# itxtx/normalizing-flows-study

Hardware: AMD Instinct MI355X
Metric: log_prob samples/sec/GPU + test-NLL match; RealNVP d=2 and MAF d=63 (higher is better)
Workload: dtype fp32

## Files before the change

normalizing-flows-study_amd/csrc/nfx_affine_kernel.h:

```cpp
#pragma once
#include <type_traits>
#include <utility>

#include "nfx_common.h"

namespace nfx {

__host__ __device__ constexpr int up4(int v) { return (v + 3) & ~3; }

struct AffineLayout {
    int d, HT, KS1;
    int w1, b1, w2, b2, w3, b3, net, mask, total;
    int s;
};

constexpr uint32_t kAffineLiveElide = 0x100u;
struct AffineSplit {
    int w1, b1, b2, w3, b3, w2s, net, mask, ok, total;
};

__host__ __device__ constexpr AffineSplit affine_split(int d, int HT) {
    AffineSplit S{};
    int o = 0;
    S.w1 = o; o += HT * ((d + 1) / 2) * 64;
    S.b1 = o; o += HT * 32;
    S.b2 = o; o += HT * 32;
    S.w3 = o; o += d * HT * 32;
// ... 101 lines not shown
                const f32x4 w = wg[a_quad(a_tile(hto, kt, HT), rq) * 64];
#pragma unroll
                for (int rr = 0; rr < 4; ++rr) {
                    a0 = mfma32(w[rr], h1[kt][0][4 * rq + rr], a0);
                    if constexpr (TILES == 2) a1 = mfma32(w[rr], h1[kt][1][4 * rq + rr], a1);
                }
            }
        }
#pragma unroll
        for (int j = 0; j < D; ++j) {
            const f32x16 w3 = load_bias16(P + L.w3 + (j * HT + hto) * 32, h);
#pragma unroll
            for (int r = 0; r < 16; ++r) {
                part[j][0] = fmaf(w3[r], trelu(a0[r]), part[j][0]);
                if constexpr (TILES == 2) part[j][1] = fmaf(w3[r], trelu(a1[r]), part[j][1]);
            }
        }
    }
#pragma unroll
    for (int j = 0; j < D; ++j)
        res[j] = tclamp(halves_sum(part[j][0], part[j][1]) + P[L.b3 + j], -10.f, 10.f);
}

#ifndef NFX_SPLIT_TERMS
#define NFX_SPLIT_TERMS 6
#endif
typedef __bf16 bf16x8 __attribute__((ext_vector_type(8)));
typedef uint32_t u32x4 __attribute__((ext_vector_type(4)));

__device__ __forceinline__ f32x16 mfma_bf16(u32x4 a, u32x4 b, f32x16 c) {
    return __builtin_amdgcn_mfma_f32_32x32x16_bf16(__builtin_bit_cast(bf16x8, a), __builtin_bit_cast(bf16x8, b), c,
                                                    0, 0, 0);
}

__device__ __forceinline__ void split3(float x, uint32_t& u0, uint32_t& u1, uint32_t& u2) {
    u0 = __float_as_uint(x) & 0xffff0000u;
    const float r1 = x - __uint_as_float(u0);
    u1 = __float_as_uint(r1) & 0xffff0000u;
    u2 = __float_as_uint(r1 - __uint_as_float(u1));
}

__device__ __forceinline__ uint32_t pack_bf16(uint32_t lo, uint32_t hi) {
    return __builtin_amdgcn_perm(hi, lo, 0x07060302u);
}

__device__ __forceinline__ void split_block(const f32x16& a, int half, u32x4 (&xp)[3]) {
#pragma unroll
    for (int q = 0; q < 4; ++q) {
        uint32_t l0, l1, l2, h0, h1, h2;
        split3(a[8 * half + 2 * q], l0, l1, l2);
        split3(a[8 * half + 2 * q + 1], h0, h1, h2);
        xp[0][q] = pack_bf16(l0, h0);
        xp[1][q] = pack_bf16(l1, h1);
        xp[2][q] = pack_bf16(l2, h2);
    }
}

template <class F, int... I>
__device__ __forceinline__ void static_for_seq(F&& f, std::integer_sequence<int, I...>) {
    (f(std::integral_constant<int, I>{}), ...);
}
template <int N, class F>
__device__ __forceinline__ void static_for(F&& f) {
    static_for_seq(f, std::make_integer_sequence<int, N>{});
}

#if NFX_SPLIT_TERMS == 8
constexpr int kSplitTermW[8] = {2, 1, 2, 1, 0, 1, 0, 0}, kSplitTermX[8] = {1, 2, 0, 1, 2, 0, 1, 0};
#else
constexpr int kSplitTermW[6] = {2, 1, 0, 1, 0, 0}, kSplitTermX[6] = {0, 1, 2, 0, 1, 0};
#endif

template <int HT, int D, int TILES, bool LIVE>
__device__ __forceinline__ void affine_nets_split_pipe(const float* __restrict__ S, const AffineSplit& SL,
                                                       const float (&xb)[2][(D + 1) / 2], float (&sv)[D],
                                                       float (&bv)[D], uint32_t live_idx) {
    constexpr int KS1 = (D + 1) / 2;
    constexpr int NJ = LIVE ? (D + 1) / 2 : D;
    constexpr int NS = 2 * TILES;
    constexpr int KB = 2 * HT;
    constexpr int NT = NFX_SPLIT_TERMS;
    constexpr int NM = NT * HT;
    constexpr int NG = KB * NM;
    constexpr int NFI = 16 * HT;
    constexpr int NQ = 3 * HT;
    constexpr int WG0 = (NM - NQ) / 2;
    constexpr int L1G = (KB - 2) * NM;
    constexpr int L1P = L1G >= 2 ? L1G - 2 : 0;
    constexpr int HB0 = NM / 2;
    const int lane = lane_id(), h = lane >> 5;

    const float* Sn[NS];
    const u32x4* w2n[NS];
    f32x16 h1[NS][HT];
// ... 565 lines not shown
```

normalizing-flows-study_amd/csrc/nfx_made.hip:

```cpp
#include "nfx_made_kernel.h"
#include "nfx_made_wide_kernel.h"
#include <atomic>
#include <cstdlib>

#include "nfx_made_seqs_kernel.h"
#include "nfx_pack.h"

namespace nfx {

__global__ void made_pack_kernel(NfxMlpRaw net, int d, int H, float* packed) {
    const int HT = (H + 31) / 32;
    const MadeLayout L = made_layout(d, HT);
    const int Hp = L.Hp, G1 = 4 * L.NKC;
    for (int i = blockIdx.x * blockDim.x + threadIdx.x; i < L.total; i += gridDim.x * blockDim.x) {
        if (i >= L.s_deg) continue;
        float v = 0.f;
        if (i < L.b1) {
            int t = i - L.w1, rr = t & 3, lane = (t >> 2) & 63, g = (t >> 8) % G1, ht = (t >> 8) / G1;
            int row = 32 * ht + (lane & 31), col = 2 * (4 * g + rr) + (lane >> 5);
            v = (row < H && col < d) ? mlp_weight(net, 0, d, row, col) : 0.f;
        } else if (i < L.w2) {
            int row = acc_vec_row(i - L.b1);
            v = row < H ? mlp_bias(net, 0, row) : 0.f;
        } else if (i < L.b2 || (i >= L.w3 && i < L.b3)) {
            const int layer = i < L.b2 ? 1 : 2;
            const ATileElem e = a_tile_elem(i - (layer == 1 ? L.w2 : L.w3));
            int row = 32 * (e.tile / HT) + e.row, col = 32 * (e.tile % HT) + e.k;
            v = (row < H && col < H) ? mlp_weight(net, layer, H, row, col) : 0.f;
// ... 85 lines not shown
        int off, word, ext;
        if (gi < n1) {
            const int ht = gi / (4 * L.NKC), g = gi % (4 * L.NKC);
            off = L.w1 + gi * 256;
            word = L.nk1 + ht;
            ext = g / 4 + 1;
        } else if (gi < n1 + 2 * n23) {
            const int t = (gi - n1) % n23, layer = (gi - n1) / n23;
            off = (layer == 0 ? L.w2 : L.w3) + t * 256;
            word = (layer == 0 ? L.nk2 : L.nk3) + t / (HT * 4);
            ext = (t % (HT * 4)) / 4 + 1;
        } else {
            const int t = gi - n1 - 2 * n23;
            off = L.w4 + t * 256;
            word = L.nk4 + t / (2 * HT * 4);
            ext = (t % (HT * 4)) / 4 + 1;
        }
        const f32x4 v = *reinterpret_cast<const f32x4*>(packed + off + 4 * lane);
        const bool nzl = v[0] != 0.f || v[1] != 0.f || v[2] != 0.f || v[3] != 0.f;
        if (__ballot(nzl) != 0 && lane == 0) atomicMax(&nk[word], ext);
    }
}

template <int HT>
made_seqs_kernel_t made_seqs_pick_ht(int variant, bool logp) {
    if (variant == NFX_MAF_FORWARD) return made_seqs_kernel<HT, NFX_MAF_FORWARD, false>;
    return logp ? made_seqs_kernel<HT, NFX_IAF_INVERSE, true> : made_seqs_kernel<HT, NFX_IAF_INVERSE, false>;
}
template made_seqs_kernel_t made_seqs_pick_ht<1>(int, bool);
template made_seqs_kernel_t made_seqs_pick_ht<2>(int, bool);

template <int HT, int VAR>
static made_seq_kernel_t seq_var() {
    return made_seq_kernel<HT, VAR>;
}

template <int HT>
made_seq_kernel_t made_seq_pick_ht(int variant) {
    return variant == NFX_MAF_FORWARD ? seq_var<HT, NFX_MAF_FORWARD>() : seq_var<HT, NFX_IAF_INVERSE>();
}
template made_seq_kernel_t made_seq_pick_ht<1>(int);
template made_seq_kernel_t made_seq_pick_ht<2>(int);
template made_seq_kernel_t made_seq_pick_ht<3>(int);
template made_seq_kernel_t made_seq_pick_ht<4>(int);

static made_par_kernel_t pick_par(int HT, bool wlds, int variant) {
    return pick_range<1, 4>(HT, [=](auto HT_) { return made_pick_ht<HT_()>(wlds, variant); });
}

static made_par_kernel_t pick_tile(int HT, bool wlds, int variant, bool logp) {
    return pick_range<1, 4>(HT, [=](auto HT_) { return made_tile_pick_ht<HT_()>(wlds, variant, logp); });
}

static made_seq_kernel_t pick_seq(int HT, int variant) {
    return pick_range<1, 4>(HT, [=](auto HT_) { return made_seq_pick_ht<HT_()>(variant); });
}

int made_big_launch(const float* packed, const float* in, float* out, float* log_det, int64_t B, int d, int H,
                    int variant, int accumulate, hipStream_t s);

constexpr size_t kLdsBytes = 160 * 1024;
constexpr int kTileMaxD = 64;

}

using namespace nfx;

extern "C" size_t nfx_made_packed_floats(int d, int H) {
    if (d <= 0 || H <= 0) return 0;
    return (size_t)made_layout(d, (H + 31) / 32).total;
}

namespace nfx {
int made_pack_seqp(int d, int H, float* packed, hipStream_t s);
static int made_pack_seq(int d, int H, float* packed, hipStream_t s) {
    const int HT = (H + 31) / 32;
    if (HT > 2) return NFX_OK;
    if (HT == 1) made_seqs_image_kernel<1><<<64, 256, 0, s>>>(packed, d, H);
    else made_seqs_image_kernel<2><<<64, 256, 0, s>>>(packed, d, H);
    int rc = check_launch("made_seqs_image_kernel");
    if (rc) return rc;
    if (HT == 1) made_seqs_chunk_kernel<1><<<1, 64, 0, s>>>(packed, d, H);
    else made_seqs_chunk_kernel<2><<<1, 64, 0, s>>>(packed, d, H);
    rc = check_launch("made_seqs_chunk_kernel");
    if (rc) return rc;
    return made_pack_seqp(d, H, packed, s);
}
}

extern "C" int nfx_made_pack_parallel(const NfxMlpRaw* net, int d, int H, float* packed, void* stream) {
    if (!net || !packed) return set_error(NFX_EINVAL, "made_pack: null pointer");
    if (d <= 0 || d > 4096 || H <= 0 || H > 256)
        return set_error(NFX_EUNSUPPORTED, "made_pack: d=%d H=%d outside d<=4096, H<=256", d, H);
    if (net->n_layers != 4) return set_error(NFX_EINVAL, "made_pack: MADE has 4 masked layers (got %d)", net->n_layers);
    for (int l = 0; l < 4; ++l)
        if (!net->w[l]) return set_error(NFX_EINVAL, "made_pack: layer %d weight is null", l);
    const int total = (int)nfx_made_packed_floats(d, H);
    int blocks = (total + 255) / 256;
    if (blocks > 2048) blocks = 2048;
    made_pack_kernel<<<blocks, 256, 0, (hipStream_t)stream>>>(*net, d, H, packed);
    int rc = check_launch("made_pack_kernel");
    if (rc) return rc;
    made_live_kernel<<<1, kLiveThreads, 0, (hipStream_t)stream>>>(*net, d, H, packed);
    rc = check_launch("made_live_kernel");
    if (rc) return rc;
    {
        const int HT = (H + 31) / 32;
        const MadeLayout L = made_layout(d, HT);
        const int groups = HT * 4 * L.NKC + 2 * HT * HT * 4 + L.NJ * 2 * HT * 4;
        made_extent_kernel<<<(groups + 3) / 4, 256, 0, (hipStream_t)stream>>>(d, H, packed);
    }
    return check_launch("made_extent_kernel");
}

extern "C" int nfx_made_pack_sequential(int d, int H, float* packed, void* stream) {
    if (!packed) return set_error(NFX_EINVAL, "made_pack_sequential: null pointer");
    if (d <= 0 || d > 4096 || H <= 0 || H > 256)
        return set_error(NFX_EUNSUPPORTED, "made_pack_sequential: d=%d H=%d outside d<=4096, H<=256", d, H);
    return made_pack_seq(d, H, packed, (hipStream_t)stream);
}

extern "C" int nfx_made_pack(const NfxMlpRaw* net, int d, int H, float* packed, void* stream) {
    const int rc = nfx_made_pack_parallel(net, d, H, packed, stream);
    if (rc) return rc;
    return made_pack_seq(d, H, packed, (hipStream_t)stream);
}

namespace nfx {
int made_seqw_launch(const float* packed, const float* in, float* out, float* log_det, int64_t B, int d, int H,
                     int variant, int accumulate, float* logp, double* partials, double* sums, bool fused,
                     int* grid_out, hipStream_t s);
int made_seqp_launch(const float* packed, const float* in, float* out, float* log_det, int64_t B, int d, int H,
                     int variant, int accumulate, float* logp, double* partials, double* sums, bool fused,
                     hipStream_t s);
}

static std::atomic<int>& made_seq_policy() {
    static std::atomic<int> v{[] {
        const char* e = getenv("NFX_MADE_SEQ_POLICY");
        return e ? atoi(e) : NFX_MADE_SEQ_AUTO;
    }()};
    return v;
}

namespace nfx {
int made_seq_policy_get() { return made_seq_policy().load(std::memory_order_relaxed); }
}

static bool tile_path(int d, int HT, int variant) {
    return (variant == NFX_MAF_INVERSE || variant == NFX_IAF_FORWARD) && d > 0 && d <= kTileMaxD && HT >= 1 && HT <= 4;
}

struct TileConfig {
    int nw;
    bool wlds;
    size_t lds;
};
static TileConfig tile_config(const MadeLayout& L, int64_t ntiles, bool fused) {
    int nw = 8;
    if (!fused && ntiles < 4 * (int64_t)num_cus()) nw = (int)((ntiles + num_cus() - 1) / num_cus());
    const size_t wbytes = (size_t)L.par_total * sizeof(float);
    const size_t tiles = nw * 32 * (size_t)kTileStride * sizeof(float);
    const bool wlds = nw == 8 && wbytes + tiles <= kLdsBytes;
    return {nw, wlds, (wlds ? wbytes : 0) + tiles};
}

static int made_launch(const float* packed, const float* in, float* out, float* log_det, int64_t B,
                       int d, int H, int variant, int accumulate, float* logp, double* sums,
                       void* workspace, hipStream_t s) {
    const bool fused = sums != nullptr;
    if (B < 0 || d <= 0 || H <= 0) return set_error(NFX_EINVAL, "made_affine: bad shape");
    if (d > 4096 || H > 256) return set_error(NFX_EUNSUPPORTED, "made_affine: d=%d H=%d outside d<=4096, H<=256", d, H);
    if (variant < NFX_MAF_INVERSE || variant > NFX_IAF_INVERSE)
        return set_error(NFX_EINVAL, "made_affine: unknown variant %d", variant);
    const int HT = (H + 31) / 32;
    if (HT > 4) {
        if (fused) return set_error(NFX_EUNSUPPORTED, "made_affine_logprob: no fused log_prob for H=%d > 128", H);
        if (B == 0) return NFX_OK;
        if (!packed || !in || !out || !log_det) return set_error(NFX_EINVAL, "made_affine: null pointer");
        if (in == out) return set_error(NFX_EINVAL, "made_affine: in and out must not alias");
        return made_big_launch(packed, in, out, log_det, B, d, H, variant, accumulate, s);
    }
    const MadeLayout L = made_layout(d, HT);
// ... 5 lines not shown
        return set_error(NFX_EUNSUPPORTED,
                         "made_affine_logprob: fused log_prob needs MAF inverse with d <= %d or H <= 64, "
                         "or IAF inverse with H <= 64", kTileMaxD);
    if (fused && B > 0 && (!logp || !workspace)) return set_error(NFX_EINVAL, "made_affine_logprob: null logp/workspace");
    if (B == 0) return fused ? gauss_finish(reinterpret_cast<double*>(workspace), 0, sums, 0, s) : NFX_OK;
    if (!packed || !in || !out || !log_det) return set_error(NFX_EINVAL, "made_affine: null pointer");
    if (in == out) return set_error(NFX_EINVAL, "made_affine: in and out must not alias");
    double* partials = reinterpret_cast<double*>(workspace);
    if (wide) {
        const int64_t nchunks = (B + 63) / 64;
        const int nw = nchunks < (int64_t)kWideWaves * num_cus() ? 4 : kWideWaves;
        const size_t lds_nw = (size_t)wide_lds(L, HT, nw).total * sizeof(float);
        made_par_kernel_t k = HT == 1 ? made_wide_pick_ht<1>(variant, fused, nw) : made_wide_pick_ht<2>(variant, fused, nw);
        int rc = prepare_lds((const void*)k, lds_nw);
        if (rc) return rc;
        int grid = resident_grid((const void*)k, 64 * nw, lds_nw, (nchunks + nw - 1) / nw);
        if (grid > kMaxPartials) grid = kMaxPartials;
        k<<<grid, 64 * nw, lds_nw, s>>>(packed, in, out, log_det, B, d, accumulate, nchunks, logp, partials,
                                        sums, gauss_const(d));
        return check_launch("made_wide_kernel");
    }
    if (tile_path(d, HT, variant)) {
        const int64_t ntiles = (B + 31) / 32;
        const TileConfig c = tile_config(L, ntiles, fused);
        made_par_kernel_t k = pick_tile(HT, c.wlds, variant, fused);
        if (!k) return set_error(NFX_EUNSUPPORTED, "made_affine: no kernel for H=%d", H);
        int rc = prepare_lds((const void*)k, c.lds);
        if (rc) return rc;
        int grid = resident_grid((const void*)k, 64 * c.nw, c.lds, (ntiles + c.nw - 1) / c.nw);
        if (grid > kMaxPartials) grid = kMaxPartials;
        k<<<grid, 64 * c.nw, c.lds, s>>>(packed, in, out, log_det, B, d, accumulate, ntiles, logp, partials, sums,
                                         gauss_const(d));
        return check_launch("made_tile_kernel");
    }
    if (variant == NFX_MAF_INVERSE || variant == NFX_IAF_FORWARD) {
        const size_t wbytes = (size_t)L.par_total * sizeof(float);
        const size_t stage8 = 8 * (size_t)kStageFloats * sizeof(float);
        const bool wlds = wbytes + stage8 <= kLdsBytes;
        made_par_kernel_t k = pick_par(HT, wlds, variant);
        if (!k) return set_error(NFX_EUNSUPPORTED, "made_affine: no kernel for H=%d", H);
        const int threads = wlds ? 512 : 256;
        const size_t lds = wlds ? wbytes + stage8 : 4 * (size_t)kStageFloats * sizeof(float);
        int rc = prepare_lds((const void*)k, lds);
        if (rc) return rc;
        const int64_t nchunks = (B + 63) / 64;
        const int nw = threads / 64;
        const int grid = resident_grid((const void*)k, threads, lds, (nchunks + nw - 1) / nw);
        k<<<grid, threads, lds, s>>>(packed, in, out, log_det, B, d, accumulate, nchunks, nullptr, nullptr, nullptr,
// ... 47 lines not shown
                                       float* logp, double* sums, void* workspace, int64_t B, int d,
                                       int H, int variant, int accumulate, void* stream) {
    if (!sums) return set_error(NFX_EINVAL, "made_affine_logprob: null sums");
    return made_launch(packed, in, out, log_det, B, d, H, variant, accumulate, logp, sums, workspace,
                       (hipStream_t)stream);
}

extern "C" int nfx_made_sample_supported(int d, int H, int variant) {
    return (H > 0 && tile_path(d, (H + 31) / 32, variant) && variant == NFX_IAF_FORWARD) ? 1 : 0;
}

extern "C" int nfx_made_affine_sample(const float* packed, uint64_t seed, uint64_t* rng_state, float* z, float* x,
                                      float* log_det, int64_t B, int d, int H, void* stream) {
    if (B < 0 || d <= 0 || H <= 0) return set_error(NFX_EINVAL, "made_affine_sample: bad shape");
    if (!nfx_made_sample_supported(d, H, NFX_IAF_FORWARD))
        return set_error(NFX_EUNSUPPORTED, "made_affine_sample: d=%d H=%d outside the tile kernel (d <= %d, H <= 128)",
                         d, H, kTileMaxD);
    if (B == 0) return NFX_OK;
    if (!packed || !rng_state || !z || !x || !log_det) return set_error(NFX_EINVAL, "made_affine_sample: null pointer");
    if (z == x) return set_error(NFX_EINVAL, "made_affine_sample: z and x must not alias");
    const int HT = (H + 31) / 32;
    const MadeLayout L = made_layout(d, HT);
    const int64_t ntiles = (B + 31) / 32;
    const TileConfig c = tile_config(L, ntiles, false);
    made_sample_kernel_t k =
        pick_range<1, 4>(HT, [=](auto HT_) { return made_tile_sample_pick_ht<HT_()>(c.wlds); });
    int rc = prepare_lds((const void*)k, c.lds);
    if (rc) return rc;
    int grid = resident_grid((const void*)k, 64 * c.nw, c.lds, (ntiles + c.nw - 1) / c.nw);
    if (grid > kMaxPartials) grid = kMaxPartials;
    k<<<grid, 64 * c.nw, c.lds, (hipStream_t)stream>>>(packed, nullptr, x, log_det, B, d, 0, ntiles, nullptr, nullptr,
                                                       nullptr, 0.f, MadeDraw{seed, rng_state, z});
    return check_launch("made_tile_kernel");
}
```

normalizing-flows-study_amd/csrc/nfx_made_kernel.h:

```cpp
#pragma once
#include "nfx_common.h"
#include "nfx_rng.h"

namespace nfx {

struct MadeLayout {
    int d, HT, Hp, NKC, NJ;
    int w1, b1, w2, b2, w3, b3, w4, b4;
    int par_total;
    int s_w1t, s_b1, s_w2, s_b2, s_w3, s_b3, s_w4, s_b4, s_deg;
    int nk1, nk2, nk3, nk4, tsafe;
    int t4, t3, t2, t1;
    int rimg;
    int sw1, sw4, sb4;
    int ctab;
    int ps, pw4, pw1, pb4, pw23, ptb, ptab;
    int total;
};

__host__ __device__ constexpr int made_up4(int v) { return (v + 3) & ~3; }

__host__ __device__ constexpr int seqs_w4_stride(int Hp) { return 2 * Hp + 4; }
constexpr int kSeqsPadRows = 64;
__host__ __device__ constexpr int seqs_max_chunks(int d, int Hp) { return d / 8 + 2 * Hp + 8; }
constexpr int kSeqpMaxS = 16;
__host__ __device__ constexpr int seqp_slots(int d, int HT) {
    return (HT <= 2 && d <= 64 * kSeqpMaxS) ? (d + 63) / 64 : 0;
}
__host__ __device__ constexpr int seqp_max_chunks(int d, int Hp) { return (d + 63) / 64 + 3 * Hp + 4; }

__host__ __device__ constexpr MadeLayout made_layout(int d, int HT) {
    MadeLayout L{};
    L.d = d;
    L.HT = HT;
    L.Hp = 32 * HT;
    L.NKC = (d + 31) / 32;
    L.NJ = (d + 31) / 32;
    int o = 0;
    L.w1 = o; o += HT * 4 * L.NKC * 256;
    L.b1 = o; o += HT * 32;
    L.w2 = o; o += HT * HT * 1024;
    L.b2 = o; o += HT * 32;
    L.w3 = o; o += HT * HT * 1024;
    L.b3 = o; o += HT * 32;
    L.w4 = o; o += L.NJ * 2 * HT * 1024;
    L.b4 = o; o += L.NJ * 2 * 32;
    L.par_total = o;
    L.s_w1t = o; o += made_up4(d * L.Hp);
    L.s_b1 = o; o += L.Hp;
    L.s_w2 = o; o += L.Hp * L.Hp;
    L.s_b2 = o; o += L.Hp;
    L.s_w3 = o; o += L.Hp * L.Hp;
// ... 10 lines not shown
    L.t4 = o; o += HT * 2 * L.NJ * 1024;
    L.t3 = o; o += HT * HT * 1024;
    L.t2 = o; o += HT * HT * 1024;
    L.t1 = o; o += L.NKC * HT * 1024;
    L.rimg = o; o += HT <= 2 ? 2 * L.Hp * L.Hp + 5 * L.Hp : 0;
    o = made_up4(o);
    const int rows = HT <= 2 ? d + kSeqsPadRows : 0;
    L.sw1 = o; o += made_up4(rows * L.Hp);
    L.sw4 = o; o += made_up4(rows * seqs_w4_stride(L.Hp));
    L.sb4 = o; o += made_up4(2 * rows);
    L.ctab = o; o += HT <= 2 ? 8 * seqs_max_chunks(d, L.Hp) : 0;
    const int PS = seqp_slots(d, HT);
    L.ps = PS;
    L.pw4 = o; o += L.Hp * ((PS + 1) / 2) * 256;
    L.pw1 = o; o += L.Hp * ((PS + 3) / 4) * 256;
    L.pb4 = o; o += PS * 128;
    L.pw23 = o; o += PS ? 2 * L.Hp * L.Hp : 0;
    L.ptb = o; o += PS ? 4 * L.Hp : 0;
    L.ptab = o; o += PS ? 16 * seqp_max_chunks(d, L.Hp) : 0;
    L.total = o;
    return L;
}

constexpr int kStageStride = 33;
constexpr int kTileStride = 65;
constexpr int kStageFloats = 64 * kStageStride;

template <int VAR>
__device__ __forceinline__ float made_affine(float xv, float mu, float al, float& acc) {
#pragma clang fp contract(off)
    if constexpr (VAR == NFX_MAF_INVERSE) {
        const float a = tclamp(al, -3.f, 3.f);
        acc = acc + a;
        const float z = (xv - mu) * exp_fast(-a);
        return nonfinite(z) ? 0.f : z;
    } else {
        const float a = tclamp(al, -2.f, 2.f);
        const float m = tclamp(mu, -10.f, 10.f);
        acc = acc + a;
        const float y = xv * exp_fast(a) + m;
        return nonfinite(y) ? xv : y;
    }
}

__device__ __forceinline__ void stage_in(const float* __restrict__ in, int64_t base, int d, int64_t B,
                                         int dim0, float* st) {
// ... 604 lines not shown
```

normalizing-flows-study_amd/csrc/nfx_tile.h:

```cpp
#pragma once

#include <hip/hip_runtime.h>

namespace nfx {

__host__ __device__ constexpr int crow(int r, int h) { return (r & 3) + 8 * (r >> 2) + 4 * h; }
__host__ __device__ constexpr int creg(int row) { return (row & 3) + 4 * (row >> 3); }
__host__ __device__ constexpr int chalf(int row) { return (row >> 2) & 1; }

struct RowCol {
    int row, col;
};

struct ATileElem {
    int tile, row, k;
};
__host__ __device__ constexpr ATileElem a_tile_elem(int t) {
    const int rr = t & 3, lane = (t >> 2) & 63, rq = (t >> 8) & 3;
    return {t >> 10, lane & 31, crow(4 * rq + rr, lane >> 5)};
}
__host__ __device__ constexpr int a_tile(int ot, int kt, int NK) { return ot * NK + kt; }
__host__ __device__ constexpr int a_quad(int tile, int rq) { return tile * 4 + rq; }

__host__ __device__ constexpr RowCol a1_elem(int t, int KS1) {
    const int lane = t & 63, ks = (t >> 6) % KS1, ht = (t >> 6) / KS1;
    return {32 * ht + (lane & 31), 2 * ks + (lane >> 5)};
}

__host__ __device__ constexpr int acc_vec_row(int t) { return 32 * (t >> 5) + crow(t & 15, (t >> 4) & 1); }

__host__ __device__ constexpr RowCol acc_dump_elem(int t) { return {crow(t >> 6, (t >> 5) & 1), t & 31}; }
__host__ __device__ constexpr int acc_dump_index(int row, int col) {
    return creg(row) * 64 + chalf(row) * 32 + col;
}
__host__ __device__ constexpr RowCol lane_dump_elem(int t) { return {crow(t & 15, (t >> 9) & 1), (t >> 4) & 31}; }

namespace tile_check {
constexpr bool crow_round_trips() {
    for (int row = 0; row < 32; ++row)
        if (crow(creg(row), chalf(row)) != row) return false;
    for (int r = 0; r < 16; ++r)
        for (int h = 0; h < 2; ++h)
            if (creg(crow(r, h)) != r || chalf(crow(r, h)) != h) return false;
    return true;
}
constexpr bool a_tile_visits_all() {
    bool seen[32 * 32] = {};
    for (int t = 0; t < 1024; ++t) {
        const ATileElem e = a_tile_elem(t);
        if (e.tile != 0 || e.row < 0 || e.row > 31 || e.k < 0 || e.k > 31 || seen[e.row * 32 + e.k]) return false;
        seen[e.row * 32 + e.k] = true;
    }
    return true;
}
constexpr bool a_tile_encode_inverts() {
    for (int t = 0; t < 3 * 1024; ++t) {
        const ATileElem e = a_tile_elem(t);
        const int r = creg(e.k), lane = e.row + 32 * chalf(e.k);
        if ((a_quad(e.tile, r >> 2) * 64 + lane) * 4 + (r & 3) != t) return false;
    }
// ... 21 lines not shown
```

Before: 1.649 billion.

## Add bf16x3 split-MFMA tile kernel for MADE with pre-split weight image

```diff
diff --git a/normalizing-flows-study_amd/csrc/nfx_affine_kernel.h b/normalizing-flows-study_amd/csrc/nfx_affine_kernel.h
--- a/normalizing-flows-study_amd/csrc/nfx_affine_kernel.h
+++ b/normalizing-flows-study_amd/csrc/nfx_affine_kernel.h
@@ -3,6 +3,7 @@
 #include <utility>
 
 #include "nfx_common.h"
+#include "nfx_split.h"
 
 namespace nfx {
 
@@ -150,39 +151,6 @@
         res[j] = tclamp(halves_sum(part[j][0], part[j][1]) + P[L.b3 + j], -10.f, 10.f);
 }
 
-#ifndef NFX_SPLIT_TERMS
-#define NFX_SPLIT_TERMS 6
-#endif
-typedef __bf16 bf16x8 __attribute__((ext_vector_type(8)));
-typedef uint32_t u32x4 __attribute__((ext_vector_type(4)));
-
-__device__ __forceinline__ f32x16 mfma_bf16(u32x4 a, u32x4 b, f32x16 c) {
-    return __builtin_amdgcn_mfma_f32_32x32x16_bf16(__builtin_bit_cast(bf16x8, a), __builtin_bit_cast(bf16x8, b), c,
-                                                    0, 0, 0);
-}
-
-__device__ __forceinline__ void split3(float x, uint32_t& u0, uint32_t& u1, uint32_t& u2) {
-    u0 = __float_as_uint(x) & 0xffff0000u;
-    const float r1 = x - __uint_as_float(u0);
-    u1 = __float_as_uint(r1) & 0xffff0000u;
-    u2 = __float_as_uint(r1 - __uint_as_float(u1));
-}
-
-__device__ __forceinline__ uint32_t pack_bf16(uint32_t lo, uint32_t hi) {
-    return __builtin_amdgcn_perm(hi, lo, 0x07060302u);
-}
-
-__device__ __forceinline__ void split_block(const f32x16& a, int half, u32x4 (&xp)[3]) {
-#pragma unroll
-    for (int q = 0; q < 4; ++q) {
-        uint32_t l0, l1, l2, h0, h1, h2;
-        split3(a[8 * half + 2 * q], l0, l1, l2);
-        split3(a[8 * half + 2 * q + 1], h0, h1, h2);
-        xp[0][q] = pack_bf16(l0, h0);
-        xp[1][q] = pack_bf16(l1, h1);
-        xp[2][q] = pack_bf16(l2, h2);
-    }
-}
 
 template <class F, int... I>
 __device__ __forceinline__ void static_for_seq(F&& f, std::integer_sequence<int, I...>) {
@@ -192,12 +160,6 @@
 __device__ __forceinline__ void static_for(F&& f) {
     static_for_seq(f, std::make_integer_sequence<int, N>{});
 }
-
-#if NFX_SPLIT_TERMS == 8
-constexpr int kSplitTermW[8] = {2, 1, 2, 1, 0, 1, 0, 0}, kSplitTermX[8] = {1, 2, 0, 1, 2, 0, 1, 0};
-#else
-constexpr int kSplitTermW[6] = {2, 1, 0, 1, 0, 0}, kSplitTermX[6] = {0, 1, 2, 0, 1, 0};
-#endif
 
 template <int HT, int D, int TILES, bool LIVE>
 __device__ __forceinline__ void affine_nets_split_pipe(const float* __restrict__ S, const AffineSplit& SL,
diff --git a/normalizing-flows-study_amd/csrc/nfx_made.hip b/normalizing-flows-study_amd/csrc/nfx_made.hip
--- a/normalizing-flows-study_amd/csrc/nfx_made.hip
+++ b/normalizing-flows-study_amd/csrc/nfx_made.hip
@@ -4,6 +4,7 @@
 #include <cstdlib>
 
 #include "nfx_made_seqs_kernel.h"
+#include "nfx_made_split_kernel.h"
 #include "nfx_pack.h"
 
 namespace nfx {
@@ -135,6 +136,74 @@
     }
 }
 
+__global__ __launch_bounds__(1024) void made_split_pack_kernel(int d, int H, float* packed) {
+    const int HT = (H + 31) / 32;
+    const MadeLayout L = made_layout(d, HT);
+    const int* nk = reinterpret_cast<const int*>(packed);
+    const MadeSplitLayout SL = made_split_layout(L);
+    int* dir = reinterpret_cast<int*>(packed) + SL.sdir;
+    uint32_t* img = reinterpret_cast<uint32_t*>(packed) + SL.simg;
+    __shared__ int sd[16];
+    __shared__ int wbad;
+    if (threadIdx.x == 0) {
+        int rows = 0;
+        for (int i = 0; i < 16; ++i) sd[i] = 0;
+        for (int ht = 0; ht < HT; ++ht) { sd[kSdirL1 + ht] = rows; rows += kSplitBlockRows * nk[L.nk1 + ht]; }
+        for (int ht = 0; ht < HT; ++ht) { sd[kSdirL2 + ht] = rows; rows += kSplitBlockRows * nk[L.nk2 + ht]; }
+        for (int ht = 0; ht < HT; ++ht) { sd[kSdirL3 + ht] = rows; rows += kSplitBlockRows * nk[L.nk3 + ht]; }
+        for (int j = 0; j < L.NJ; ++j)
+            for (int which = 0; which < 2; ++which) {
+                sd[kSdirL4 + 2 * j + which] = rows;
+                rows += kSplitBlockRows * nk[L.nk4 + j];
+            }
+        sd[kSdirRows] = rows;
+        wbad = 0;
+    }
+    __syncthreads();
+    const int n1 = HT * L.NKC, n23 = HT * HT, n4 = 2 * L.NJ * HT;
+    constexpr int kBlk = kSplitBlockRows * kSplitRowDwords;
+    bool bad = false;
+    for (int i = threadIdx.x; i < (n1 + 2 * n23 + n4) * kBlk; i += blockDim.x) {
+        const int blk = i / kBlk, t = i % kBlk;
+        int ot, kt, ext, first, src;
+        if (blk < n1) {
+            ot = blk / L.NKC, kt = blk % L.NKC;
+            ext = nk[L.nk1 + ot], first = sd[kSdirL1 + ot], src = -1;
+        } else if (blk < n1 + 2 * n23) {
+            const int b = (blk - n1) % n23, layer = (blk - n1) / n23;
+            ot = b / HT, kt = b % HT;
+            ext = nk[(layer ? L.nk3 : L.nk2) + ot], first = sd[(layer ? kSdirL3 : kSdirL2) + ot];
+            src = (layer ? L.w3 : L.w2) + a_tile(ot, kt, HT) * 1024;
+        } else {
+            const int b = blk - n1 - 2 * n23;
+            ot = b / HT, kt = b % HT;
+            ext = nk[L.nk4 + (ot >> 1)], first = sd[kSdirL4 + ot];
+            src = L.w4 + a_tile(ot, kt, HT) * 1024;
+        }
+        if (kt >= ext) continue;
+        uint32_t half[2];
+        for (int e = 0; e < 2; ++e) {
+            const SplitElem s = split_elem(t, e, src >= 0);
+            const float w = src >= 0 ? packed[src + a_tile_index(0, s.row, s.k)]
+                                     : packed[L.w1 + a1q_index(ot, s.row, 32 * kt + s.k, 4 * L.NKC)];
+            if (!(fabsf(w) <= 1e6f) || (w != 0.f && fabsf(w) < 0x1p-100f)) bad = true;
+            const uint32_t u0 = __builtin_bit_cast(uint16_t, (__bf16)w);
+            const float r1 = w - __uint_as_float(u0 << 16);
+            const uint32_t u1 = __builtin_bit_cast(uint16_t, (__bf16)r1);
+            const uint32_t u2 = __builtin_bit_cast(uint16_t, (__bf16)(r1 - __uint_as_float(u1 << 16)));
+            half[e] = s.piece == 0 ? u0 : s.piece == 1 ? u1 : u2;
+        }
+        img[(first + kSplitBlockRows * kt) * kSplitRowDwords + t] = half[0] | (half[1] << 16);
+    }
+    if (bad) atomicOr(&wbad, 1);
+    __syncthreads();
+    if (threadIdx.x < 16) {
+        int v = sd[threadIdx.x];
+        if (threadIdx.x == kSdirSafe) v = __float_as_int(wbad ? 0.f : packed[L.tsafe]);
+        dir[threadIdx.x] = v;
+    }
+}
+
 template <int HT>
 made_seqs_kernel_t made_seqs_pick_ht(int variant, bool logp) {
     if (variant == NFX_MAF_FORWARD) return made_seqs_kernel<HT, NFX_MAF_FORWARD, false>;
@@ -165,6 +234,13 @@
     return pick_range<1, 4>(HT, [=](auto HT_) { return made_tile_pick_ht<HT_()>(wlds, variant, logp); });
 }
 
+static made_par_kernel_t pick_tile_split(bool wlds, int variant, bool logp) {
+    if (variant == NFX_MAF_INVERSE) return wlds ? made_tile_split_maf_pick<true>(logp) : made_tile_split_maf_pick<false>(logp);
+    return wlds ? made_tile_split_iaf_pick<true>() : made_tile_split_iaf_pick<false>();
+}
+
+constexpr bool kMadeSplitDefault = true;
+
 static made_seq_kernel_t pick_seq(int HT, int variant) {
     return pick_range<1, 4>(HT, [=](auto HT_) { return made_seq_pick_ht<HT_()>(variant); });
 }
@@ -181,7 +257,7 @@
 
 extern "C" size_t nfx_made_packed_floats(int d, int H) {
     if (d <= 0 || H <= 0) return 0;
-    return (size_t)made_layout(d, (H + 31) / 32).total;
+    return (size_t)made_split_layout(made_layout(d, (H + 31) / 32)).total;
 }
 
 namespace nfx {
@@ -222,8 +298,11 @@
         const MadeLayout L = made_layout(d, HT);
         const int groups = HT * 4 * L.NKC + 2 * HT * HT * 4 + L.NJ * 2 * HT * 4;
         made_extent_kernel<<<(groups + 3) / 4, 256, 0, (hipStream_t)stream>>>(d, H, packed);
-    }
-    return check_launch("made_extent_kernel");
+        rc = check_launch("made_extent_kernel");
+        if (rc || !made_has_split(d, HT)) return rc;
+        made_split_pack_kernel<<<1, 1024, 0, (hipStream_t)stream>>>(d, H, packed);
+    }
+    return check_launch("made_split_pack_kernel");
 }
 
 extern "C" int nfx_made_pack_sequential(int d, int H, float* packed, void* stream) {
@@ -269,9 +348,16 @@
     bool wlds;
     size_t lds;
 };
-static TileConfig tile_config(const MadeLayout& L, int64_t ntiles, bool fused) {
+static bool made_split_on(int d, int HT) {
+    if (!made_has_split(d, HT)) return false;
+    const char* e = getenv("NFX_MADE_SPLIT");
+    return e ? atoi(e) != 0 : kMadeSplitDefault;
+}
+
+static TileConfig tile_config(const MadeLayout& L, int64_t ntiles, bool fused, bool split = false) {
     int nw = 8;
     if (!fused && ntiles < 4 * (int64_t)num_cus()) nw = (int)((ntiles + num_cus() - 1) / num_cus());
+    if (split) return {nw, nw == 8, nw == 8 ? (size_t)kSplitLdsBytes : nw * 32 * (size_t)kTileStride * sizeof(float)};
     const size_t wbytes = (size_t)L.par_total * sizeof(float);
     const size_t tiles = nw * 32 * (size_t)kTileStride * sizeof(float);
     const bool wlds = nw == 8 && wbytes + tiles <= kLdsBytes;
@@ -323,8 +409,9 @@
     }
     if (tile_path(d, HT, variant)) {
         const int64_t ntiles = (B + 31) / 32;
-        const TileConfig c = tile_config(L, ntiles, fused);
-        made_par_kernel_t k = pick_tile(HT, c.wlds, variant, fused);
+        const bool split = made_split_on(d, HT);
+        const TileConfig c = tile_config(L, ntiles, fused, split);
+        made_par_kernel_t k = split ? pick_tile_split(c.wlds, variant, fused) : pick_tile(HT, c.wlds, variant, fused);
         if (!k) return set_error(NFX_EUNSUPPORTED, "made_affine: no kernel for H=%d", H);
         int rc = prepare_lds((const void*)k, c.lds);
         if (rc) return rc;
@@ -418,9 +505,11 @@
     const int HT = (H + 31) / 32;
     const MadeLayout L = made_layout(d, HT);
     const int64_t ntiles = (B + 31) / 32;
-    const TileConfig c = tile_config(L, ntiles, false);
+    const bool split = made_split_on(d, HT);
+    const TileConfig c = tile_config(L, ntiles, false, split);
     made_sample_kernel_t k =
-        pick_range<1, 4>(HT, [=](auto HT_) { return made_tile_sample_pick_ht<HT_()>(c.wlds); });
+        split ? (c.wlds ? made_tile_split_sample_pick<true>() : made_tile_split_sample_pick<false>())
+              : pick_range<1, 4>(HT, [=](auto HT_) { return made_tile_sample_pick_ht<HT_()>(c.wlds); });
     int rc = prepare_lds((const void*)k, c.lds);
     if (rc) return rc;
     int grid = resident_grid((const void*)k, 64 * c.nw, c.lds, (ntiles + c.nw - 1) / c.nw);
diff --git a/normalizing-flows-study_amd/csrc/nfx_made_kernel.h b/normalizing-flows-study_amd/csrc/nfx_made_kernel.h
--- a/normalizing-flows-study_amd/csrc/nfx_made_kernel.h
+++ b/normalizing-flows-study_amd/csrc/nfx_made_kernel.h
@@ -28,6 +28,9 @@
     return (HT <= 2 && d <= 64 * kSeqpMaxS) ? (d + 63) / 64 : 0;
 }
 __host__ __device__ constexpr int seqp_max_chunks(int d, int Hp) { return (d + 63) / 64 + 3 * Hp + 4; }
+
+__host__ __device__ constexpr bool made_has_split(int d, int HT) { return HT == 2 && d > 32 && d <= 64; }
+constexpr int kSplitRowDwords = 256, kSplitBlockRows = 6;
 
 __host__ __device__ constexpr MadeLayout made_layout(int d, int HT) {
     MadeLayout L{};
@@ -84,6 +87,19 @@
     return L;
 }
 
+struct MadeSplitLayout {
+    int sdir, simg, total;
+};
+__host__ __device__ constexpr MadeSplitLayout made_split_layout(const MadeLayout& L) {
+    MadeSplitLayout S{};
+    int o = made_up4(L.total);
+    const bool SP = made_has_split(L.d, L.HT);
+    S.sdir = o; o += SP ? 16 : 0;
+    S.simg = o; o += SP ? (L.HT * L.NKC + 2 * L.HT * L.HT + 2 * L.NJ * L.HT) * kSplitBlockRows * kSplitRowDwords : 0;
+    S.total = o;
+    return S;
+}
+
 constexpr int kStageStride = 33;
 constexpr int kTileStride = 65;
 constexpr int kStageFloats = 64 * kStageStride;
diff --git a/normalizing-flows-study_amd/csrc/nfx_made_split.hip b/normalizing-flows-study_amd/csrc/nfx_made_split.hip
--- /dev/null
+++ b/normalizing-flows-study_amd/csrc/nfx_made_split.hip
@@ -0,0 +1,15 @@
+#include "nfx_made_split_kernel.h"
+
+namespace nfx {
+
+template <bool WLDS>
+made_par_kernel_t made_tile_split_maf_pick(bool logp) {
+    if constexpr (WLDS) {
+        if (logp) return made_tile_split_kernel<2, true, NFX_MAF_INVERSE, true>;
+    }
+    return made_tile_split_kernel<2, WLDS, NFX_MAF_INVERSE, false>;
+}
+template made_par_kernel_t made_tile_split_maf_pick<true>(bool);
+template made_par_kernel_t made_tile_split_maf_pick<false>(bool);
+
+}
diff --git a/normalizing-flows-study_amd/csrc/nfx_made_split_iaf.hip b/normalizing-flows-study_amd/csrc/nfx_made_split_iaf.hip
--- /dev/null
+++ b/normalizing-flows-study_amd/csrc/nfx_made_split_iaf.hip
@@ -0,0 +1,19 @@
+#include "nfx_made_split_kernel.h"
+
+namespace nfx {
+
+template <bool WLDS>
+made_par_kernel_t made_tile_split_iaf_pick() {
+    return made_tile_split_kernel<2, WLDS, NFX_IAF_FORWARD, false>;
+}
+template made_par_kernel_t made_tile_split_iaf_pick<true>();
+template made_par_kernel_t made_tile_split_iaf_pick<false>();
+
+template <bool WLDS>
+made_sample_kernel_t made_tile_split_sample_pick() {
+    return made_tile_split_kernel<2, WLDS, NFX_IAF_FORWARD, false, true, MadeDraw>;
+}
+template made_sample_kernel_t made_tile_split_sample_pick<true>();
+template made_sample_kernel_t made_tile_split_sample_pick<false>();
+
+}
diff --git a/normalizing-flows-study_amd/csrc/nfx_made_split_kernel.h b/normalizing-flows-study_amd/csrc/nfx_made_split_kernel.h
--- /dev/null
+++ b/normalizing-flows-study_amd/csrc/nfx_made_split_kernel.h
@@ -0,0 +1,320 @@
+#pragma once
+#include "nfx_made_kernel.h"
+#include "nfx_split.h"
+
+namespace nfx {
+
+enum MadeSplitDir {
+    kSdirL1 = 0,
+    kSdirL2 = 2,
+    kSdirL3 = 4,
+    kSdirL4 = 6,
+    kSdirRows = 10,
+    kSdirSafe = 11,
+};
+
+constexpr int kSplitLdsBytes = 160 * 1024 - 512;
+__host__ __device__ constexpr int split_bias_floats(int HT, int NJ) { return 3 * HT * 32 + NJ * 64; }
+
+__device__ __forceinline__ void split_lin_block(const float* xr, u32x4 (&xp)[3]) {
+#pragma unroll
+    for (int q = 0; q < 4; ++q) {
+        uint32_t l0, l1, l2, h0, h1, h2;
+        split3(xr[2 * q], l0, l1, l2);
+        split3(xr[2 * q + 1], h0, h1, h2);
+        xp[0][q] = pack_bf16(l0, h0);
+        xp[1][q] = pack_bf16(l1, h1);
+        xp[2][q] = pack_bf16(l2, h2);
+    }
+}
+
+template <bool FIRST>
+__device__ __forceinline__ void split_terms(const u32x4* w, const u32x4 (&xp)[3], f32x16& hi, f32x16& lo) {
+    const u32x4 wp[3] = {w[0], w[64], w[128]};
+#pragma unroll
+    for (int t = 0; t < NFX_SPLIT_TERMS - 1; ++t)
+        lo = mfma_bf16(wp[kSplitTermW[t]], xp[kSplitTermX[t]], FIRST && t == 0 ? f32x16{} : lo);
+    hi = mfma_bf16(wp[0], xp[0], hi);
+}
+
+template <int NKB>
+__device__ __forceinline__ f32x16 split_tile(const u32x4* im, int first, int nkb, const float* bias,
+                                             const u32x4 (&xp)[NKB][3]) {
+    f32x16 hi = load_bias16(bias, lane_id() >> 5), lo;
+    if (nkb <= 0) return hi;
+    split_terms<true>(im + first * 64, xp[0], hi, lo);
+#pragma unroll
+    for (int kb = 1; kb < NKB; ++kb)
+        if (kb < nkb) split_terms<false>(im + (first + 3 * kb) * 64, xp[kb], hi, lo);
+    return hi + lo;
+}
+
+template <int NO, int NKB>
+__device__ __forceinline__ void split_layer(const u32x4* im, const int (&first)[NO], const int (&nkb)[NO],
+                                            const float* bias, const u32x4 (&xp)[NKB][3], f32x16 (&hout)[NO]) {
+#pragma unroll
+    for (int o = 0; o < NO; ++o) {
+        const f32x16 a = split_tile<NKB>(im, first[o], nkb[o], bias + o * 32, xp);
+#pragma unroll
+        for (int r = 0; r < 16; ++r) hout[o][r] = trelu(a[r]);
+    }
+}
+
+template <int HT, bool STAGED, int VAR, bool LOGP, bool SAMPLE, typename... DRAW>
+__device__ __forceinline__ void made_split_run(const float* __restrict__ packed, const float* __restrict__ in,
+                                               float* __restrict__ out, float* __restrict__ logdet, int64_t B, int d,
+                                               int accumulate, int64_t ntiles, float* __restrict__ logp, float cgauss,
+                                               float* lds, int nwg, double& lpacc, DRAW... draw) {
+    const MadeLayout L = made_layout(d, HT);
+    constexpr int S = kTileStride;
+    const int wave = __builtin_amdgcn_readfirstlane(threadIdx.x >> 6);
+    float* xt = lds + wave * 32 * S;
+    const int lane = lane_id(), h = lane >> 5, col = lane & 31;
+    const int64_t nwaves = (int64_t)gridDim.x * nwg;
+    const int voff = lane < d ? lane * 4 : (1 << 30);
+    const int rowb = d * 4;
+    const int* nkp = reinterpret_cast<const int*>(packed);
+    const MadeSplitLayout SL = made_split_layout(L);
+    const int* dirp = nkp + SL.sdir;
+    int nkb1[HT], nkb2[HT], nkb3[HT], f1[HT], f2[HT], f3[HT];
+#pragma unroll
+    for (int i = 0; i < HT; ++i) {
+        nkb1[i] = 2 * nkp[L.nk1 + i];
+        nkb2[i] = 2 * nkp[L.nk2 + i];
+        nkb3[i] = 2 * nkp[L.nk3 + i];
+        f1[i] = dirp[kSdirL1 + i];
+        f2[i] = dirp[kSdirL2 + i];
+        f3[i] = dirp[kSdirL3 + i];
+    }
+    const float ssafe = __int_as_float(dirp[kSdirSafe]);
+    const bool allbad = !(ssafe > 0.f);
+    const float* bb = STAGED ? lds + 8 * 32 * S : packed;
+    const int ob1 = STAGED ? 0 : L.b1, ob2 = STAGED ? HT * 32 : L.b2, ob3 = STAGED ? 2 * HT * 32 : L.b3,
+              ob4 = STAGED ? 3 * HT * 32 : L.b4;
+    const u32x4* img = (STAGED ? reinterpret_cast<const u32x4*>(lds + 8 * 32 * S + split_bias_floats(HT, L.NJ))
+                               : reinterpret_cast<const u32x4*>(packed + SL.simg)) + lane;
+
+    int64_t t = (int64_t)blockIdx.x * nwg + wave;
+    float pf[32];
+    float ldpf = 0.f;
+    uint64_t draw_off = 0;
+    auto fetch = [&](int64_t tn) {
+        if constexpr (SAMPLE) {
+            made_draw_tile(pf, tn, ntiles, B, d, made_draw_arg(draw...).seed, draw_off);
+        } else {
+            ldpf = (accumulate && tn < ntiles && lane < 32 && tn * 32 + col < B) ? logdet[tn * 32 + col] : 0.f;
+            const int64_t rn = tn < ntiles ? (B - tn * 32 < 32 ? B - tn * 32 : 32) : 0;
+            const auto rs = __builtin_amdgcn_make_buffer_rsrc(const_cast<float*>(in) + (tn < ntiles ? tn * 32 * d : 0), 0,
+                                                              (int)(rn * rowb), 0x00020000);
+#pragma unroll
+            for (int r = 0; r < 32; ++r)
+                pf[r] = __uint_as_float(__builtin_amdgcn_raw_buffer_load_b32(rs, voff, r * rowb, 0));
+        }
+    };
+    if constexpr (SAMPLE) draw_off = rng_offset(made_draw_arg(draw...).rng);
+    fetch(t);
+    for (; t < ntiles; t += nwaves) {
+        const int64_t base = t * 32;
+        const int rows = (int)(B - base < 32 ? B - base : 32);
+        const u32x4* im = img + opaque_zero();
+        const float* bz = bb + opaque_zero();
+        float xmax = 0.f;
+#pragma unroll
+        for (int r = 0; r < 32; ++r) {
+            xt[r * S + lane] = pf[r];
+            xmax = tmax(xmax, fabsf(pf[r]));
+        }
+        if constexpr (SAMPLE) {
+            const auto rs = __builtin_amdgcn_make_buffer_rsrc(made_draw_arg(draw...).z + base * d, 0, rows * rowb,
+                                                              0x00020000);
+#pragma unroll
+            for (int r = 0; r < 32; ++r)
+                __builtin_amdgcn_raw_buffer_store_b32(__float_as_uint(pf[r]), rs, voff, r * rowb, 0);
+        }
+        const bool anybad = allbad || __builtin_amdgcn_ballot_w64(!(xmax <= ssafe)) != 0;
+        wave_lds_sync();
+        const float ldin = ldpf;
+        float acc = 0.f;
+
+        if (!allbad) {
+            f32x16 h1[HT], h2[HT];
+            {
+                u32x4 xp[4][3];
+#pragma unroll
+                for (int kb = 0; kb < 4; ++kb)
+                    split_lin_block(xt + col * S + split_lin_k(kb & 1, h, 0) + 32 * (kb >> 1), xp[kb]);
+                split_layer<HT, 4>(im, f1, nkb1, bz + ob1, xp, h1);
+            }
+            {
+                u32x4 xp[2 * HT][3];
+#pragma unroll
+                for (int kb = 0; kb < 2 * HT; ++kb) split_block(h1[kb >> 1], kb & 1, xp[kb]);
+                split_layer<HT, 2 * HT>(im, f2, nkb2, bz + ob2, xp, h2);
+            }
+            u32x4 xp[2 * HT][3];
+            {
+#pragma unroll
+                for (int kb = 0; kb < 2 * HT; ++kb) split_block(h2[kb >> 1], kb & 1, xp[kb]);
+                split_layer<HT, 2 * HT>(im, f3, nkb3, bz + ob3, xp, h1);
+            }
+#pragma unroll
+            for (int kb = 0; kb < 2 * HT; ++kb) split_block(h1[kb >> 1], kb & 1, xp[kb]);
+
+            if (!anybad) fetch(t + nwaves);
+
+            for (int j = 0; j < L.NJ; ++j) {
+                const int n4 = 2 * nkp[L.nk4 + j], fm = dirp[kSdirL4 + 2 * j], fa = dirp[kSdirL4 + 2 * j + 1];
+                const f32x16 mu = split_tile<2 * HT>(im, fm, n4, bz + ob4 + (j * 2 + 0) * 32, xp);
+                const f32x16 alv = split_tile<2 * HT>(im, fa, n4, bz + ob4 + (j * 2 + 1) * 32, xp);
+#pragma unroll
+                for (int r = 0; r < 16; ++r) {
+                    float* p = xt + col * S + 32 * j + crow(r, h);
+                    *p = made_affine<VAR>(*p, mu[r], alv[r], acc);
+                }
+            }
+            wave_lds_sync();
+        }
+        if (anybad) {
+            uint32_t badmask = 0xffffffffu;
+            if (!allbad) {
+                fetch(t);
+                badmask = 0;
+#pragma unroll
+                for (int r = 0; r < 32; ++r)
+                    if (__builtin_amdgcn_ballot_w64(!(fabsf(pf[r]) <= ssafe)) != 0) badmask |= 1u << r;
+#pragma unroll
+                for (int r = 0; r < 32; ++r)
+                    if ((badmask >> r) & 1) xt[r * S + lane] = pf[r];
+                wave_lds_sync();
+            }
+            const bool badcol = (badmask >> col) & 1;
+            const float* W = packed + opaque_zero();
+            f32x16 g1[HT], g2[HT];
+#pragma unroll
+            for (int ht = 0; ht < HT; ++ht) {
+                f32x16 a = load_bias16(W + L.b1 + ht * 32, h);
+                for (int kc = 0; kc < L.NKC; ++kc) {
+#pragma unroll
+                    for (int g = 0; g < 4; ++g) {
+                        const f32x4 w =
+                            *reinterpret_cast<const f32x4*>(W + L.w1 + ((ht * 4 * L.NKC + kc * 4 + g) * 64 + lane) * 4);
+#pragma unroll
+                        for (int rr = 0; rr < 4; ++rr) a = mfma32(w[rr], xt[col * S + 32 * kc + 8 * g + 2 * rr + h], a);
+                    }
+                }
+#pragma unroll
+                for (int r = 0; r < 16; ++r) a[r] = trelu(a[r]);
+                g1[ht] = a;
+            }
+            made_hidden1<HT>(W, L.w2, L.b2, g1, g2);
+            made_hidden1<HT>(W, L.w3, L.b3, g2, g1);
+            float acc2 = 0.f;
+            for (int j = 0; j < L.NJ; ++j) {
+                f32x16 mu, al;
+                out_pair<HT, HT>(W, L, j, g1, mu, al);
+#pragma unroll
+                for (int r = 0; r < 16; ++r) {
+                    float* p = xt + col * S + 32 * j + crow(r, h);
+                    const float v = made_affine<VAR>(*p, mu[r], al[r], acc2);
+                    if (badcol) *p = v;
+                }
+            }
+            acc = badcol ? acc2 : acc;
+            wave_lds_sync();
+            fetch(t + nwaves);
+        }
+
+        const float ssum = halves_sum(acc, acc);
+        float zsq = 0.f;
+        if constexpr (LOGP) {
+            if (lane < 32) {
+                for (int jd = 0; jd < d; ++jd) {
+                    const float v = xt[col * S + jd];
+                    zsq = (jd == 0) ? gauss_sq0(v) : gauss_sq(zsq, v);
+                }
+            }
+        }
+        {
+            const auto rs = __builtin_amdgcn_make_buffer_rsrc(out + base * d, 0, rows * rowb, 0x00020000);
+#pragma unroll
+            for (int r = 0; r < 32; ++r)
+                __builtin_amdgcn_raw_buffer_store_b32(__float_as_uint(xt[r * S + lane]), rs, voff, r * rowb, 0);
+        }
+        if (lane < 32 && col < rows) {
+            float ldv;
+            if constexpr (VAR == NFX_MAF_INVERSE) {
+                ldv = -ssum;
+                if (nonfinite(ldv)) ldv = 0.f;
+                ldv = tclamp(ldv, -100.f, 100.f);
+            } else {
+                ldv = ssum;
+                if (nonfinite(ldv)) ldv = 0.f;
+                ldv = tclamp(ldv, -50.f, 50.f);
+            }
+            const int64_t so = base + col;
+            const float ldt = accumulate ? ldin + ldv : ldv;
+            logdet[so] = ldt;
+            if constexpr (LOGP) {
+                const float lp = gauss_lp(zsq, cgauss, ldt);
+                logp[so] = lp;
+                lpacc += (double)lp;
+            }
+        }
+        wave_lds_sync();
+    }
+}
+
+template <int HT, bool WLDS, int VAR, bool LOGP, bool SAMPLE = false, typename... DRAW>
+__global__ __launch_bounds__(512) void made_tile_split_kernel(
+    const float* __restrict__ packed, const float* __restrict__ in, float* __restrict__ out,
+    float* __restrict__ logdet, int64_t B, int d, int accumulate, int64_t ntiles,
+    float* __restrict__ logp, double* __restrict__ partials, double* __restrict__ sums, float cgauss,
+    DRAW... draw) {
+    static_assert(sizeof...(DRAW) == (SAMPLE ? 1 : 0), "SAMPLE kernels take one MadeDraw");
+    static_assert(!SAMPLE || (VAR == NFX_IAF_FORWARD && !LOGP), "SAMPLE: the IAF forward pass");
+    extern __shared__ f32x4 lds4[];
+    float* lds = reinterpret_cast<float*>(lds4);
+    double lpacc = 0.0;
+    if constexpr (WLDS) {
+        const MadeLayout L = made_layout(d, HT);
+        const MadeSplitLayout SL = made_split_layout(L);
+        const int crows = reinterpret_cast<const int*>(packed)[SL.sdir + kSdirRows];
+        const int nb = split_bias_floats(HT, L.NJ);
+        const int head = 8 * 32 * kTileStride + nb;
+        const bool fits = (head + crows * kSplitRowDwords) * 4 <= kSplitLdsBytes;
+        if (fits) {
+            float* bl = lds + 8 * 32 * kTileStride;
+            for (int i = threadIdx.x; i < nb; i += 512) {
+                const int l = i / (HT * 32);
+                bl[i] = l < 3 ? packed[(l == 0 ? L.b1 : l == 1 ? L.b2 : L.b3) + i - l * HT * 32] : packed[L.b4 + i - 3 * HT * 32];
+            }
+            const f32x4* src = reinterpret_cast<const f32x4*>(packed + SL.simg);
+            f32x4* dst = reinterpret_cast<f32x4*>(lds + head);
+            for (int i = threadIdx.x; i < crows * 64; i += 512) dst[i] = src[i];
+            __syncthreads();
+            made_split_run<HT, true, VAR, LOGP, SAMPLE>(packed, in, out, logdet, B, d, accumulate, ntiles, logp, cgauss,
+                                                        lds, 8, lpacc, draw...);
+        } else {
+            made_split_run<HT, false, VAR, LOGP, SAMPLE>(packed, in, out, logdet, B, d, accumulate, ntiles, logp, cgauss,
+                                                         lds, 8, lpacc, draw...);
+        }
+    } else {
+        made_split_run<HT, false, VAR, LOGP, SAMPLE>(packed, in, out, logdet, B, d, accumulate, ntiles, logp, cgauss, lds,
+                                                     (int)(blockDim.x >> 6), lpacc, draw...);
+    }
+    if constexpr (LOGP) {
+        logp_commit<512>(lpacc, partials, sums, B);
+    }
+    if constexpr (SAMPLE) {
+        rng_commit(made_draw_arg(draw...).rng);
+    }
+}
+
+template <bool WLDS>
+made_par_kernel_t made_tile_split_maf_pick(bool logp);
+template <bool WLDS>
+made_par_kernel_t made_tile_split_iaf_pick();
+template <bool WLDS>
+made_sample_kernel_t made_tile_split_sample_pick();
+
+}
diff --git a/normalizing-flows-study_amd/csrc/nfx_split.h b/normalizing-flows-study_amd/csrc/nfx_split.h
--- /dev/null
+++ b/normalizing-flows-study_amd/csrc/nfx_split.h
@@ -0,0 +1,46 @@
+#pragma once
+#include "nfx_common.h"
+
+namespace nfx {
+
+#ifndef NFX_SPLIT_TERMS
+#define NFX_SPLIT_TERMS 6
+#endif
+typedef __bf16 bf16x8 __attribute__((ext_vector_type(8)));
+typedef uint32_t u32x4 __attribute__((ext_vector_type(4)));
+
+__device__ __forceinline__ f32x16 mfma_bf16(u32x4 a, u32x4 b, f32x16 c) {
+    return __builtin_amdgcn_mfma_f32_32x32x16_bf16(__builtin_bit_cast(bf16x8, a), __builtin_bit_cast(bf16x8, b), c,
+                                                    0, 0, 0);
+}
+
+__device__ __forceinline__ void split3(float x, uint32_t& u0, uint32_t& u1, uint32_t& u2) {
+    u0 = __float_as_uint(x) & 0xffff0000u;
+    const float r1 = x - __uint_as_float(u0);
+    u1 = __float_as_uint(r1) & 0xffff0000u;
+    u2 = __float_as_uint(r1 - __uint_as_float(u1));
+}
+
+__device__ __forceinline__ uint32_t pack_bf16(uint32_t lo, uint32_t hi) {
+    return __builtin_amdgcn_perm(hi, lo, 0x07060302u);
+}
+
+__device__ __forceinline__ void split_block(const f32x16& a, int half, u32x4 (&xp)[3]) {
+#pragma unroll
+    for (int q = 0; q < 4; ++q) {
+        uint32_t l0, l1, l2, h0, h1, h2;
+        split3(a[8 * half + 2 * q], l0, l1, l2);
+        split3(a[8 * half + 2 * q + 1], h0, h1, h2);
+        xp[0][q] = pack_bf16(l0, h0);
+        xp[1][q] = pack_bf16(l1, h1);
+        xp[2][q] = pack_bf16(l2, h2);
+    }
+}
+
+#if NFX_SPLIT_TERMS == 8
+constexpr int kSplitTermW[8] = {2, 1, 2, 1, 0, 1, 0, 0}, kSplitTermX[8] = {1, 2, 0, 1, 2, 0, 1, 0};
+#else
+constexpr int kSplitTermW[6] = {2, 1, 0, 1, 0, 0}, kSplitTermX[6] = {0, 1, 2, 0, 1, 0};
+#endif
+
+}
diff --git a/normalizing-flows-study_amd/csrc/nfx_tile.h b/normalizing-flows-study_amd/csrc/nfx_tile.h
--- a/normalizing-flows-study_amd/csrc/nfx_tile.h
+++ b/normalizing-flows-study_amd/csrc/nfx_tile.h
@@ -35,7 +35,61 @@
 }
 __host__ __device__ constexpr RowCol lane_dump_elem(int t) { return {crow(t & 15, (t >> 9) & 1), (t >> 4) & 31}; }
 
+__host__ __device__ constexpr int a_tile_index(int tile, int row, int k) {
+    return (a_quad(tile, creg(k) >> 2) * 64 + row + 32 * chalf(k)) * 4 + (creg(k) & 3);
+}
+
+__host__ __device__ constexpr int a1q_index(int ht, int row, int col, int G1) {
+    return ((ht * G1 + (col >> 3)) * 64 + row + 32 * (col & 1)) * 4 + ((col >> 1) & 3);
+}
+__host__ __device__ constexpr RowCol a1q_elem(int t, int G1) {
+    const int rr = t & 3, lane = (t >> 2) & 63, g = (t >> 8) % G1, ht = (t >> 8) / G1;
+    return {32 * ht + (lane & 31), 2 * (4 * g + rr) + (lane >> 5)};
+}
+
+struct SplitElem {
+    int kb, piece, row, k, e;
+};
+__host__ __device__ constexpr int split_acc_k(int kb, int h, int j) { return crow(8 * kb + j, h); }
+__host__ __device__ constexpr int split_lin_k(int kb, int h, int j) { return 16 * kb + 8 * h + j; }
+__host__ __device__ constexpr SplitElem split_elem(int t, int e, bool acc) {
+    const int q = t & 3, lane = (t >> 2) & 63, g = t >> 8;
+    const int kb = g / 3, j = 2 * q + e;
+    return {kb, g % 3, lane & 31, acc ? split_acc_k(kb, lane >> 5, j) : split_lin_k(kb, lane >> 5, j), e};
+}
+__host__ __device__ constexpr int split_index(int piece, int row, int k, bool acc) {
+    const int kb = acc ? creg(k) >> 3 : k >> 4, h = acc ? chalf(k) : (k >> 3) & 1, j = (acc ? creg(k) : k) & 7;
+    return (((kb * 3 + piece) * 64) + row + 32 * h) * 4 + (j >> 1);
+}
+
 namespace tile_check {
+constexpr bool split_round_trips(bool acc) {
+    for (int t = 0; t < 1536; ++t)
+        for (int e = 0; e < 2; ++e) {
+            const SplitElem s = split_elem(t, e, acc);
+            if (s.row < 0 || s.row > 31 || s.k < 0 || s.k > 31) return false;
+            if (split_index(s.piece, s.row, s.k, acc) != t || ((acc ? creg(s.k) : s.k) & 1) != e) return false;
+        }
+    return true;
+}
+constexpr bool a1q_round_trips() {
+    for (int G1 = 4; G1 <= 8; G1 += 4)
+        for (int t = 0; t < 2 * G1 * 256; ++t) {
+            const RowCol e = a1q_elem(t, G1);
+            if (a1q_index(e.row >> 5, e.row & 31, e.col, G1) != t) return false;
+        }
+    return true;
+}
+constexpr bool a_tile_index_inverts() {
+    for (int t = 0; t < 3 * 1024; ++t) {
+        const ATileElem e = a_tile_elem(t);
+        if (a_tile_index(e.tile, e.row, e.k) != t) return false;
+    }
+    return true;
+}
+static_assert(split_round_trips(true) && split_round_trips(false), "split block encode inverts the decode");
+static_assert(a1q_round_trips(), "MADE layer-1 encode inverts the decode");
+static_assert(a_tile_index_inverts(), "a_tile_index inverts a_tile_elem");
 constexpr bool crow_round_trips() {
     for (int row = 0; row < 32; ++row)
         if (crow(creg(row), chalf(row)) != row) return false;
```

Result: no change. 1.648 billion (-0.0%).
